# kakaoenterprise/JORLDY

Measured on NVIDIA H100. Metric: env_steps_per_sec, higher is better.
Workload: dtype f32

## Files before the change

include/jorldy_b200.h:

```cpp
#ifndef JORLDY_B200_H
#define JORLDY_B200_H

#include <stdint.h>

#ifdef __cplusplus
#define JB_API extern "C"
#else
#define JB_API
#endif

JB_API int jb_env_classic_reset(int kind, double* phys, float* obs, int32_t* elapsed, int64_t* episode,
                                float* score, const uint8_t* mask, uint64_t seed, uint64_t stream_base,
                                int n, void* stream);
JB_API int jb_env_classic_step(int kind, double* phys, float* obs, int32_t* elapsed, int64_t* episode,
                               float* score, const void* action, int action_kind, float* next_obs,
                               float* reward, float* done, float* stats, int auto_reset, int max_steps,
                               uint64_t seed, uint64_t stream_base, int n, void* stream);

JB_API int jb_gae(const float* reward, const float* done, const float* value, const float* next_value,
                  const float* last_value, int N, int T, float gamma, float lambda, int standardize,
                  float* adv, float* ret, void* stream);

JB_API int
jb_env_synth_reset(float* obs, int32_t* elapsed, int64_t* episode, float* score, uint64_t seed,
// ... 60 lines not shown
                           float* db1, int n1, float* dw2, float* db2, int n2, void* stream);

JB_API int jb_ppo_act_discrete(const float* out, int M, int A, int nout, const float* u, uint64_t seed,
                               uint64_t stream_base, uint64_t ctr, long long* row_ctr, int greedy, int64_t* action,
                               void* stream);
JB_API int jb_ppo_act_continuous(const float* out, int M, int A, int nout, const float* normal, uint64_t seed,
                                 uint64_t stream_base, uint64_t ctr, long long* row_ctr, int greedy, float* action,
                                 void* stream);
JB_API int jb_ppo_prepass_discrete(const float* out, const int32_t* action, int M, int A, int nout, float* value,
                                   float* logp_old, void* stream);
JB_API int jb_ppo_prepass_continuous(const float* out, const float* action, int M, int A, int nout, float* value,
                                     float* logp_old, void* stream);
JB_API int jb_take_minibatch(const int32_t* perm, long long* cursor, int B, int32_t* cur_idx, void* stream);
JB_API int jb_ppo_loss(int continuous, const float* out, const int32_t* idx, const void* action, const float* adv,
                       const float* ret, const float* value_old, const float* logp_old, int B, int A, int nout,
                       float eps_clip, float vf_coef, float ent_coef, float* dout, float* stats, float* acc,
                       void* stream);

JB_API int jb_env_frames_reset(uint8_t* obs, int64_t* fcount, float* score, uint64_t seed, uint64_t stream_base, int n,
                               void* stream);
JB_API int jb_env_frames_step(uint8_t* obs, int64_t* fcount, float* score, uint8_t* next_obs, float* reward, float* done,
                              float* stats, int auto_reset, uint64_t seed, uint64_t stream_base, int n, void* stream);

JB_API int jb_im2col_u8(const uint8_t* x, int B, int C, int H, int W, int KH, int KW, int S, float* col, void* stream);
JB_API int jb_im2col_nhwc(const float* x, int B, int C, int H, int W, int KH, int KW, int S, float* col, void* stream);
JB_API int jb_col2im_nhwc(const float* dcol, int B, int C, int H, int W, int KH, int KW, int S, const float* relu_act,
                          float* dx, void* stream);
JB_API int jb_nhwc_to_nchw(const float* x, int B, int P, int C, float* y, void* stream);
JB_API int jb_nchw_to_nhwc(const float* x, int B, int P, int C, const float* relu_act, float* y, void* stream);

JB_API int jb_ppo_fused_args_size(void);
JB_API int jb_ppo_fused_max_ctas(void);
JB_API int jb_ppo_fused_run(const void* host_args, void* stream);
JB_API int jb_ppo_fused_trace(long long* host_out);

JB_API int jb_q_act(const float* q, int M, int A, float eps, const float* eps_rows, const float* u, uint64_t seed,
                    uint64_t stream_base, long long* row_ctr, int64_t* action, float* q_sel, void* stream);
JB_API int jb_dueling_fwd(const float* adv, const float* val, int B, int A, int K, float* out, void* stream);
JB_API int jb_dueling_bwd(const float* dout, int B, int A, int K, float* dadv, float* dval, void* stream);
JB_API int jb_td_loss(const float* q, const float* q_next, const float* qt_next, const void* action, int action_kind,
                      const float* reward, const float* done, const double* weights, int B, int A, float gamma,
                      float alpha, int n_step, int double_q, int loss_kind, int order, float* dq, double* prio,
                      float* stats, void* stream);

JB_API int jb_c51_loss(const float* logits, const float* next_online, const float* next_target, const void* action,
                       int action_kind, const float* reward, const float* done, const double* weights, const float* z,
                       int B, int A, int K, float gamma, float v_min, float v_max, float alpha, int n_step, int variant,
                       float* dlogits, float* kl, double* prio, float* stats, float* scratch, void* stream);
JB_API int jb_c51_q(const float* logits, const float* z, int M, int A, int K, float* q, void* stream);

JB_API int jb_noisy_make(const float* mu_w, const float* sig_w, const float* mu_b, const float* sig_b, int in_f,
                         int out_f, const float* eps_i, const float* eps_j, uint64_t seed, uint64_t stream_id,
                         long long* draw_ctr, int is_train, float* f_i, float* f_j, float* w_eff, float* b_eff,
                         void* stream);
JB_API int jb_noisy_grad(const float* dw_eff, const float* db_eff, const float* f_i, const float* f_j, int in_f,
                         int out_f, float* dmu_w, float* dsig_w, float* dmu_b, float* dsig_b, void* stream);

JB_API int jb_grad_partials_count(long long P);
JB_API int jb_grad_sumsq(const float* g, long long P, float* partials, long long* step, void* stream);
JB_API int jb_adam_step(float* p, const float* g, float* m, float* v, long long P, const float* lr, double beta1,
                        double beta2, float eps, const long long* step, const float* partials, int n_partials,
                        float max_norm, float* norm_out, void* stream);
JB_API int jb_rmsprop_centered_step(float* p, const float* g, float* square_avg, float* grad_avg, long long P,
                                    const float* lr, double alpha, float eps, const float* partials, int n_partials,
                                    float max_norm, float* norm_out, void* stream);
JB_API int jb_copy_f32(float* dst, const float* src, long long P, void* stream);
// ... 67 lines not shown
```

jorldy_b200/csrc/ppo_fused.cu:

```cuda
#include <cstdlib>
#include "common.cuh"
#include "ppo_rowmath.cuh"
#include "wgmma.cuh"
#include "../../include/jorldy_b200_fused.h"

namespace {

constexpr int NT = 256;
constexpr int PK = 512;
constexpr int MAXD = 16;
constexpr int MAXO = 8;
constexpr int KG = 16;
constexpr int SMALL_FLOATS = 2048;
constexpr int RED_FLOATS = KG * (32 * 36 + 16);
constexpr int JA_ROWS = 256;
constexpr int R2_FLOATS = JA_ROWS * 32;
constexpr int MAX_B = 512;
constexpr int ADAM_IT = 4;
constexpr int PS_FLOATS = (MAXO + 2) * PK;
constexpr int CTR_ROW = 1;
constexpr int CTR_JB = 32;

typedef jb_ppo_fused_args Args;

__device__ __forceinline__ float ldcg(const float* p) { return __ldcg(p); }
__device__ __forceinline__ float4 ldcg4(const float* p) { return __ldcg(reinterpret_cast<const float4*>(p)); }

__device__ __forceinline__ unsigned smem_u32(const void* p) { return (unsigned)__cvta_generic_to_shared(p); }
__device__ __forceinline__ void cp_async4(float* dst, const void* src) {
  asm volatile("cp.async.ca.shared.global [%0], [%1], 4;\n" ::"r"(smem_u32(dst)), "l"(src) : "memory");
}
struct Stager {
  unsigned mbar;
  unsigned bytes;
  unsigned parity;
  __device__ __forceinline__ void init(void* bar) {
    mbar = smem_u32(bar); bytes = 0; parity = 0;
    if (threadIdx.x == 0) {
      asm volatile("mbarrier.init.shared::cta.b64 [%0], 1;\n" ::"r"(mbar) : "memory");
      asm volatile("fence.mbarrier_init.release.cluster;\n" ::: "memory");
    }
  }
  __device__ __forceinline__ void copy(void* dst, const void* src, unsigned nbytes) const {
    asm volatile("cp.async.bulk.shared::cluster.global.mbarrier::complete_tx::bytes [%0], [%1], %2, [%3];\n"
                 ::"r"(smem_u32(dst)), "l"(src), "r"(nbytes), "r"(mbar) : "memory");
  }
  __device__ __forceinline__ void commit() {
    if (bytes && threadIdx.x == 0)
      asm volatile("mbarrier.arrive.expect_tx.shared::cta.b64 _, [%0], %1;\n" ::"r"(mbar), "r"(bytes) : "memory");
    bytes = 0;
  }
  __device__ __forceinline__ void wait() {
    asm volatile(
        "{\n\t"
// ... 217 lines not shown
        "mbarrier.try_wait.parity.shared::cta.b64 p, [%1], %2;\n\t"
        "selp.u32 %0, 1, 0, p;\n\t"
        "}\n" : "=r"(done) : "r"(mbar), "r"(parity) : "memory");
    if (done) return;
    if (clock64() - t0 > (1ll << 32)) asm volatile("trap;\n");
  }
}
__device__ __forceinline__ void mbar_expect_tx(unsigned mbar, unsigned bytes) {
  asm volatile("mbarrier.arrive.expect_tx.shared::cta.b64 _, [%0], %1;\n" ::"r"(mbar), "r"(bytes) : "memory");
}
__device__ __forceinline__ void bulk_g2s(unsigned dst, const void* src, unsigned bytes, unsigned mbar) {
  asm volatile("cp.async.bulk.shared::cluster.global.mbarrier::complete_tx::bytes [%0], [%1], %2, [%3];\n"
               ::"r"(dst), "l"(src), "r"(bytes), "r"(mbar) : "memory");
}
__device__ __forceinline__ float tf32_lo(float x) {
  const float r = x - __uint_as_float(__float_as_uint(x) & 0xFFFFE000u);
  unsigned o;
  asm("cvt.rna.tf32.f32 %0, %1;\n" : "=r"(o) : "f"(r));
  return __uint_as_float(o);
}
constexpr int TC_A_BYTES = 2 * 128 * 128;
constexpr int TC_B_BYTES = 2 * 32 * 128;
constexpr int TC_NA = 3, TC_NB = 5;
constexpr int TC_BAR_WORD = 1664;
constexpr int TC_BAR_JB = TC_NB;
constexpr int TC_NBAR = TC_NB + TC_NA;
constexpr int TC_LD = 36;

__device__ long long g_trace[256 * 48];
#define TR(i) do { if (trace && tid == 0) g_trace[cta * 48 + (i)] = clock64(); } while (0)

struct HeadTab { const float* w[MAXO]; const float* b[MAXO]; float* gw[MAXO]; float* gb[MAXO]; };

template <bool TC, int NA, int ND>
__global__ void __launch_bounds__(NT, 1) ppo_epoch_kernel(Args a, int dsm_floats, int flags ) {
  extern __shared__ __align__(16) float smem[];
  float* s_small = smem;
  float* dsm = smem + SMALL_FLOATS;
  float* R0 = dsm + dsm_floats;
  float* R1 = R0 + RED_FLOATS;
  float* R2 = R1 + RED_FLOATS;
  float* PS = R2 + R2_FLOATS;
  float* xs = s_small;
  float* scr = s_small + 768;
  int* sidx = reinterpret_cast<int*>(s_small + 1024);
  Stager st;
  st.init(s_small + 1056);
  Stager stp;
  stp.init(s_small + 1058);
  float* dvs = s_small + 1088;
  float* hb = s_small + 1600;
  unsigned tc_base = 0;
  unsigned long long tc_g = 0;
  unsigned long long jb_g = 0;
  unsigned long long ja_g = 0;
  const unsigned tc_bar = smem_u32(s_small + TC_BAR_WORD);
  float* tcp = nullptr;
  float* tcs = nullptr;

  const int tid = threadIdx.x, lane = tid & 31, warp = tid >> 5, wg = tid >> 7;
  const unsigned int nctas = gridDim.x;
  const int cta = blockIdx.x;
  const int B = a.B, D = a.D, H = a.H, A = a.A, nout = a.nout;
  const int npol = a.continuous ? 2 * A : A;
  constexpr int NO = 2 * NA + 1 < MAXO ? 2 * NA + 1 : MAXO;
  const int nq = (nout + 3) >> 2;
  const float invB = 1.0f / (float)B;
  const jbppo::HP hp{a.eps_clip, a.vf_coef, a.ent_coef};
  unsigned int epoch = 0;
  const long long step0 = *a.step, cursor0 = *a.cursor;
  const float lr = *a.lr;

  if (TC) {
    tc_base = (smem_u32(R0) + 1023u) & ~1023u;
    tcp = R0 + ((tc_base - smem_u32(R0)) >> 2);
    tcs = tcp + TC_A_BYTES / 4;
    if (tid == 0) {
      for (int i = 0; i < TC_NBAR; ++i) mbar_init(tc_bar + 8u * i, 1);
      asm volatile("fence.mbarrier_init.release.cluster;\n" ::: "memory");
    }
    __syncthreads();
  }
  HeadTab& ht = *reinterpret_cast<HeadTab*>(s_small + 896);
  if (tid == 0) {
    int o = 0;
    for (int g = 0; g < 3; ++g)
      for (int q = 0; q < a.nh[g]; ++q, ++o) {
        ht.w[o] = a.Wh[g] + (size_t)q * H; ht.b[o] = a.bh[g] + q; ht.gw[o] = a.gWh[g] + (size_t)q * H; ht.gb[o] = a.gbh[g] + q;
      }
    for (; o < MAXO; ++o) { ht.w[o] = a.Wh[0]; ht.b[o] = a.bh[0]; ht.gw[o] = a.gWh[0]; ht.gb[o] = a.gbh[0]; }
  }
  __syncthreads();

  const int MT = B / 32, NTL = H / 32, NP = (NTL + 1) >> 1;
  const int nJ1 = TC ? (B >> 7) * NTL : MT * NTL;
  const int nJB = TC ? (H >> 7) * MT : MT * NTL;
  const int nJA = TC ? (H >> 7) * NTL : NTL * NP;
  const int nJC = NTL;
  const int nJD = NTL;
  const int nJ3 = nJB + nJA + nJC + nJD;
  const bool single = B <= JA_ROWS;

  const long long per = (a.P4 + nctas - 1) / nctas;
  const long long lo = (long long)cta * per, hi = min(a.P4, lo + per);
  float4* p4 = reinterpret_cast<float4*>(a.flat);
  const float4* g4 = reinterpret_cast<const float4*>(a.grad);
  float4* m4 = reinterpret_cast<float4*>(a.am);
  float4* v4 = reinterpret_cast<float4*>(a.av);
  double pw1 = pow((double)a.beta1, (double)(step0 + 1)), pw2 = pow((double)a.beta2, (double)(step0 + 1));
  const long long w2_lo = (long long)(a.W2 - a.flat) >> 2, w2_hi = w2_lo + (long long)H * H / 4;
  auto shadow = [&](long long i, float4 v) {
    if (i >= w2_lo && i < w2_hi) {
      const int e = (int)(i - w2_lo) * 4, n = e / H, k = e - n * H;
      *reinterpret_cast<float4*>(&a.W2t[((size_t)(k >> 5) * H + n) * 32 + (k & 31)]) = v;
      if (TC) {
        float* img = a.W2img + ((size_t)(n >> 5) * (H >> 5) + (k >> 5)) * 1024 + (tile_off(n & 31, (k & 31) >> 2) >> 2);
        *reinterpret_cast<float4*>(img) = v;
        *reinterpret_cast<float4*>(img + (size_t)H * H) = make_float4(tf32_lo(v.x), tf32_lo(v.y), tf32_lo(v.z), tf32_lo(v.w));
        const float vv4[4] = {v.x, v.y, v.z, v.w};
#pragma unroll
        for (int q = 0; q < 4; ++q) {
          const int kk = k + q;
          float* t = a.W2Timg + ((size_t)(kk >> 7) * (H >> 5) + (n >> 5)) * 4096 + (tile_off(kk & 127, (n & 31) >> 2) >> 2) + (n & 3);
          t[0] = vv4[q];
          t[(size_t)H * H] = tf32_lo(vv4[q]);
        }
      }
    }
  };
  for (long long i = lo + tid; i < hi; i += NT) shadow(i, p4[i]);
  const float one_m_b1 = 1.f - a.beta1, one_m_b2 = 1.f - a.beta2;

  auto issue_stage = [&](int job, bool b_in_flight) {
    if (job < nJB) {
// ... 329 lines not shown
      tile_reduce<true, true>(acc, R0, outv);
      TR(4);
      {
        float v[4];
#pragma unroll
        for (int r = 0; r < 4; ++r) {
          v[r] = fmaxf(outv[r] + b2v, 0.f);
          a.h2[(size_t)(m0 + warp + 8 * r) * H + n0 + lane] = v[r];
          a.h2t[((size_t)nt * B + m0 + warp + 8 * r) * 32 + lane] = v[r];
        }
        float hv_[16];
        const bool up16 = (lane & 16) != 0;
#pragma unroll
        for (int q = 0; q < 16; ++q) hv_[q] = butterfly_pair(v[q / MAXO] * whr[q % MAXO], v[q / MAXO + 2] * whr[q % MAXO], up16, 16);
        butterfly_level<8>(hv_, lane);
        butterfly_level<4>(hv_, lane);
        butterfly_level<2>(hv_, lane);
        butterfly_level<1>(hv_, lane);
        TR(35);
        const int r = lane >> 3, o = lane & 7;
        if (o < 4 * nq) a.headp[(((size_t)nt * 2 + (o >> 2)) * B + m0 + warp + 8 * r) * 4 + (o & 3)] = o < nout ? hv_[0] : 0.f;
      }
      row_ticket(mt, tid < 32, m0 + tid, tid);
    }
    xs_ready = false;
    TR(5);
    grid_bar(a.barrier, epoch, nctas);
    TR(6);

    stp.bytes = (unsigned)B * (MAXO + 1) * 4u;
    stp.commit();
    if (tid == 0) { stp.copy(dsm, a.dout, (unsigned)B * MAXO * 4u); stp.copy(dvs, a.dv2, (unsigned)B * 4u); }
    int pre_job = -1;
    if (cta < nJ3 && (cta < nJB || prefetchable(cta))) { issue_stage(cta, w2t_pre); pre_job = cta; }
    auto jb_issue_a = [&](int kt4, int nc, unsigned long long g) {
      const unsigned slot = (unsigned)(g % TC_NA);
      const unsigned bar = tc_bar + 8u * (TC_BAR_JB + slot), dst = tc_base + slot * TC_A_BYTES;
      mbar_expect_tx(bar, TC_A_BYTES);
      const float* src = a.W2Timg + ((size_t)kt4 * (H >> 5) + nc) * 4096;
      bulk_g2s(dst, src, 16384u, bar);
      bulk_g2s(dst + 16384u, src + (size_t)H * H, 16384u, bar);
    };
    if (TC && cta >= nJB && cta < nJB + nJA) {
      for (int e = tid; e < B * D; e += NT) { const int m = e / D, i = e - m * D; R2[i * B + m] = ldcg(a.xg + e); }
    }
    if (TC && cta < nJB && tid == 0) {
      jb_issue_a(cta / MT, 0, jb_g);
      if ((H >> 5) > 1) jb_issue_a(cta / MT, 1, jb_g + 1);
    }
    const bool has_next = (s + 1 < a.n_steps) && cta < nJ1;
    int next_r = 0;
    if (TC) { if (has_next) next_r = a.perm[(cursor0 + s + 1) * (long long)B + (cta / NTL) * 128 + (tid & 127)]; }
    else if (has_next && tid < 32) next_r = a.perm[(cursor0 + s + 1) * (long long)B + (cta / NTL) * 32 + tid];

    float c1, c2;
    {
      float p1 = 0.f, p2 = 0.f, ssum = 0.f, esum = 0.f, mr = -INFINITY, mp = INFINITY;
#pragma unroll 1
      for (int b = tid; b < B; b += NT) {
        const float d1 = ldcg(a.rowst + b), d2 = ldcg(a.rowst + B + b);
        p1 = fmaf(d1, d1, p1); p2 = fmaf(d2, d2, p2);
        ssum += ldcg(a.rowst + 2 * B + b); esum += ldcg(a.rowst + 3 * B + b);
        mr = fmaxf(mr, ldcg(a.rowst + 4 * B + b)); mp = fminf(mp, ldcg(a.rowst + 5 * B + b));
      }
      p1 = jb_warp_sum(p1); p2 = jb_warp_sum(p2); ssum = jb_warp_sum(ssum); esum = jb_warp_sum(esum);
      mr = jb_warp_max(mr); mp = jb_warp_min(mp);
      if (lane == 0) { float* q = scr + warp * 8; q[0] = p1; q[1] = p2; q[2] = ssum; q[3] = esum; q[4] = mr; q[5] = mp; }
// ... 36 lines not shown
          scr[96 + 2 * tid + 1] = __uint_as_float((unsigned int)m2);
        }
        __syncthreads();
        TR(40);
        float g1 = 0.f, g2 = 0.f;
        for (int r = 0; r < a.world; ++r) {
          g1 += r == a.rank ? t1 : scr[96 + 2 * r];
          g2 += r == a.rank ? t2 : scr[96 + 2 * r + 1];
        }
        t1 = g1; t2 = g2;
        invBW = invB / (float)a.world;
      }
      c1 = t1 * invBW; c2 = t2 * invBW;
      float w1, w2;
      jbppo::critic_weights(c1, c2, w1, w2);
      stp.wait();
      TR(38);
      for (int b = tid; b < B; b += NT) dsm[b * MAXO + npol] = w1 * dsm[b * MAXO + npol] + w2 * dvs[b];
      if (cta == (int)nctas - 1 && tid == 0) {
        float s3 = 0.f, s4 = 0.f, xr = -INFINITY, xp = INFINITY;
        for (int w = 0; w < NT / 32; ++w) { s3 += scr[w * 8 + 2]; s4 += scr[w * 8 + 3]; xr = fmaxf(xr, scr[w * 8 + 4]); xp = fminf(xp, scr[w * 8 + 5]); }
        a.acc[0] += -s3 * invB;
        a.acc[1] += fmaxf(c1, c2);
        a.acc[2] += -s4 * invB / (a.continuous ? (float)A : 1.f);
        a.acc[3] = fmaxf(a.acc[3], xr);
        a.acc[4] = fminf(a.acc[4], xp);
        a.acc[5] += 1.f;
      }
      __syncthreads();
    }
    TR(7);

    float sq = 0.f;
    for (int job = cta; job < nJ3; job += (int)nctas) {
      __syncthreads();
      TR(8 + min(3, (job - cta) / (int)nctas));
      const int next = job + (int)nctas;
      if (TC && job < nJB) {
        const int kt4 = job / MT, mt = job - kt4 * MT, m0 = mt * 32, kin0 = kt4 * 128, NKC = H >> 5;
        if (job != cta && tid == 0) {
          jb_issue_a(kt4, 0, jb_g);
          if (NKC > 1) jb_issue_a(kt4, 1, jb_g + 1);
        }
        for (int e = tid; e < 32 * MAXD; e += NT) { const int r = e >> 4, i = e & 15; xs[i * 32 + r] = i < D ? ldcg(a.xg + (size_t)(m0 + r) * D + i) : 0.f; }
        const int ml = tid >> 3, c8 = tid & 7;
        const float* drow = &dsm[(m0 + ml) * MAXO];
        float4 hq = ldcg4(a.h2 + (size_t)(m0 + ml) * H + 4 * c8);
        float acc[16];
        for (int nc = 0; nc < NKC; ++nc) {
          const unsigned long long g = jb_g + nc;
          const unsigned slot = (unsigned)(g % TC_NA);
          float4 wr[MAXO];
#pragma unroll
          for (int o = 0; o < MAXO; ++o) wr[o] = o < nout ? *reinterpret_cast<const float4*>(&PS[o * PK + nc * 32 + 4 * c8]) : make_float4(0.f, 0.f, 0.f, 0.f);
          const float4 hcur = hq;
          if (nc + 1 < NKC) hq = ldcg4(a.h2 + (size_t)(m0 + ml) * H + (nc + 1) * 32 + 4 * c8);
          const float4 dv = dh2_quad<NO>(drow, wr, hcur);
          const float4 lo = make_float4(tf32_lo(dv.x), tf32_lo(dv.y), tf32_lo(dv.z), tf32_lo(dv.w));
          const unsigned bbuf = tc_base + TC_NA * TC_A_BYTES + slot * TC_B_BYTES, off = tile_off(ml, c8);
          asm volatile("st.shared.v4.f32 [%0], {%1, %2, %3, %4};\n" ::"r"(bbuf + off), "f"(dv.x), "f"(dv.y), "f"(dv.z), "f"(dv.w) : "memory");
          asm volatile("st.shared.v4.f32 [%0], {%1, %2, %3, %4};\n" ::"r"(bbuf + 4096u + off), "f"(lo.x), "f"(lo.y), "f"(lo.z), "f"(lo.w) : "memory");
          jbwg::wait<0>();
          jbwg::fence_acc(acc);
          asm volatile("fence.proxy.async.shared::cta;\n" ::: "memory");
          __syncthreads();
          if (tid == 0 && nc + 2 < NKC) jb_issue_a(kt4, nc + 2, g + 2);
          mbar_wait(tc_bar + 8u * (TC_BAR_JB + slot), (unsigned)((g / TC_NA) & 1));
          const unsigned aw = tc_base + slot * TC_A_BYTES + (unsigned)wg * 8192u;
          jbwg::fence();
          jbwg::mma3_n32(acc, aw, aw + 16384u, bbuf, bbuf + 4096u, nc == 0);
          jbwg::commit();
        }
        jbwg::wait<0>();
        jbwg::fence_acc(acc);
        __syncthreads();
        jbwg::store_acc_n32(acc, tcs, TC_LD);
        __syncthreads();
        if (prefetchable(next)) { issue_stage(next, false); pre_job = next; }
        {
          const int q = warp & 3, cb = (warp >> 2) * 16, kin = kin0 + q * 32 + lane;
          float rr[16];
#pragma unroll
          for (int c = 0; c < 4; ++c) {
            const float4 t = *reinterpret_cast<const float4*>(&tcs[(q * 32 + lane) * TC_LD + cb + 4 * c]);
            rr[4 * c] = t.x; rr[4 * c + 1] = t.y; rr[4 * c + 2] = t.z; rr[4 * c + 3] = t.w;
          }
          float w1r[ND];
#pragma unroll
          for (int i = 0; i < ND; ++i) w1r[i] = i < D ? ldcg(a.W1 + (size_t)kin * D + i) : 0.f;
          const float b1v = PS[(MAXO + 1) * PK + kin];
          float wacc[ND + 1];
#pragma unroll
          for (int i = 0; i <= ND; ++i) wacc[i] = 0.f;
#pragma unroll
          for (int j = 0; j < 16; ++j) {
            const int ml2 = cb + j;
            float h = 0.f;
#pragma unroll
            for (int i = 0; i < ND; ++i) if (i < D) h = fmaf(xs[i * 32 + ml2], w1r[i], h);
            const float dvv = (h + b1v > 0.f) ? rr[j] : 0.f;
#pragma unroll
            for (int i = 0; i < ND; ++i) if (i < D) wacc[i] = fmaf(dvv, xs[i * 32 + ml2], wacc[i]);
            wacc[ND] += dvv;
          }
          float* sc = tcp + (size_t)(q * 32 + lane) * (MAXD + 1);
          if (warp >= 4) {
#pragma unroll
            for (int i = 0; i <= ND; ++i) if (i < D || i == ND) sc[i < D ? i : MAXD] = wacc[i];
          }
          __syncthreads();
          if (warp < 4) {
// ... 9 lines not shown
        jb_g += (unsigned long long)NKC;
        TR(16);
      } else if (!TC && job < nJB) {
        const int mt = job / NTL, kt = job - mt * NTL;
        const int m0 = mt * 32, k0 = kt * 32;
        if (pre_job != job) issue_stage(job, false);
        const int c4 = (tid & 127) * 4, rh = tid >> 7;
        float4 wr[MAXO];
#pragma unroll
        for (int o = 0; o < MAXO; ++o)
          wr[o] = (o < nout && c4 < H) ? *reinterpret_cast<const float4*>(&PS[o * PK + c4]) : make_float4(0.f, 0.f, 0.f, 0.f);
        if (TC || !(job == cta && nJ1 <= (int)nctas))
          for (int e = tid; e < 32 * MAXD; e += NT) { const int r = e >> 4, i = e & 15; xs[i * 32 + r] = i < D ? ldcg(a.xg + (size_t)(m0 + r) * D + i) : 0.f; }
        float h1m[4];
#pragma unroll
        for (int r = 0; r < 4; ++r)
          asm volatile("ld.global.cg.f32 %0, [%1];\n" : "=f"(h1m[r]) : "l"(a.h1 + ((size_t)kt * B + m0 + warp + 8 * r) * 32 + lane));
        st.wait();
        TR(12);
        if (c4 < H) {
#pragma unroll 4
          for (int r = 0; r < 16; ++r) {
            const int row = rh * 16 + r;
            float4* pa = reinterpret_cast<float4*>(&R0[row * (H + 4) + c4]);
            *pa = dh2_quad<NO>(&dsm[(m0 + row) * MAXO], wr, *pa);
          }
        }
        __syncthreads();
        TR(13);
        float acc[8][8] = {};
        tile_mma<true, false>(R0, R1, H, acc, nullptr);
        __syncthreads();
        TR(14);
        if (prefetchable(next)) { issue_stage(next, false); pre_job = next; }
        float outv[4];
        tile_reduce<true, false>(acc, R0, outv);
        TR(15);
        float wacc[MAXD + 1];
#pragma unroll
        for (int i = 0; i <= MAXD; ++i) wacc[i] = 0.f;
#pragma unroll
        for (int r = 0; r < 4; ++r) {
          const float dv = h1m[r] > 0.f ? outv[r] : 0.f;
          const float* xrow = &xs[warp + 8 * r];
#pragma unroll
          for (int i = 0; i < MAXD; ++i) if (i < D) wacc[i] = fmaf(dv, xrow[i * 32], wacc[i]);
          wacc[MAXD] += dv;
        }
        __syncthreads();
#pragma unroll
        for (int i = 0; i <= MAXD; ++i) if (i < D || i == MAXD) R0[(warp * (MAXD + 1) + i) * 32 + lane] = wacc[i];
        __syncthreads();
        TR(33);
        for (int e = tid; e < 32 * (D + 1); e += NT) {
          const int n = e / (D + 1), i = e - n * (D + 1);
          const int slot = i < D ? i : MAXD;
          float t = R0[(0 * (MAXD + 1) + slot) * 32 + n];
#pragma unroll
          for (int w = 1; w < NT / 32; ++w) t += R0[(w * (MAXD + 1) + slot) * 32 + n];
          a.w1p[((size_t)mt * H + k0) * (D + 1) + e] = t;
        }
        __syncthreads();
        TR(34);
        if (tid == 0) asm volatile("red.release.gpu.global.add.u32 [%0], 1;\n" ::"l"(a.barrier + CTR_JB + kt) : "memory");
        TR(16);
      } else if (TC && job < nJB + nJA) {
        const int j = job - nJB, kt4 = j / NTL, nt = j - kt4 * NTL, k0 = kt4 * 128, n0 = nt * 32, NMC = B >> 5;
// ... 113 lines not shown
        float4 wr[MAXO];
#pragma unroll
        for (int o = 0; o < MAXO; ++o) wr[o] = o < nout ? *reinterpret_cast<const float4*>(&PS[o * PK + n0 + 4 * cg]) : make_float4(0.f, 0.f, 0.f, 0.f);
        const int nhalf = (kt0 + 1 < NTL) ? 2 : 1;
        for (int half = 0; half < nhalf; ++half) {
          const int kt = kt0 + half, k0 = kt * 32;
          const float* Bp = R1 + ((single && half == 1) ? R2_FLOATS : 0);
          float acc[8][8] = {};
          float rs[8] = {0.f, 0.f, 0.f, 0.f, 0.f, 0.f, 0.f, 0.f};
          for (int mp = 0; mp < B; mp += JA_ROWS) {
            const int kp = min(JA_ROWS, B - mp);
            if (!single || half == 0) {
              if (single) {
                if (pre_job != job) issue_stage(job, false);
              } else {
                __syncthreads();
                stage_block(st, R2, a.h2t + ((size_t)nt * B + mp) * 32, kp);
                stage_block(st, R1, a.h1 + ((size_t)kt * B + mp) * 32, kp);
                st.commit();
              }
              st.wait();
              TR(17);
              for (int m = rl; m < kp; m += 32) {
                float4* pa = reinterpret_cast<float4*>(&R2[m * 32 + 4 * cg]);
                *pa = dh2_quad<NO>(&dsm[(mp + m) * MAXO], wr, *pa);
              }
              __syncthreads();
              TR(18);
            }
            tile_mma<false, false>(R2, Bp, kp, acc, kt == 0 ? rs : nullptr);
          }
          __syncthreads();
          TR(19);
          if (half == nhalf - 1 && prefetchable(next)) { issue_stage(next, false); pre_job = next; }
          float outv[4];
          tile_reduce<false, false>(acc, R0, outv);
          TR(20);
#pragma unroll
          for (int r = 0; r < 4; ++r) {
            a.gW2[(size_t)(n0 + warp + 8 * r) * H + k0 + lane] = outv[r];
            sq = fmaf(outv[r], outv[r], sq);
          }
          if (kt == 0) {
            const int grp = tid >> 4, t = tid & 15, tx = t & 3, ty = t >> 2;
            __syncthreads();
            if (tx == 0) {
#pragma unroll
              for (int i = 0; i < 8; ++i) R0[grp * 32 + ty * 8 + i] = rs[i];
            }
            __syncthreads();
            if (tid < 32) {
              float v = 0.f;
#pragma unroll
              for (int g = 0; g < KG; ++g) v += R0[g * 32 + tid];
              a.gb2[n0 + tid] = v;
              sq = fmaf(v, v, sq);
            }
            __syncthreads();
          }
        }
        TR(21);
      } else if (job < nJB + nJA + nJC) {
        const int jt = job - nJB - nJA;
        const int j0 = jt * 32;
        float hacc[MAXO];
#pragma unroll
        for (int o = 0; o < MAXO; ++o) hacc[o] = 0.f;
        for (int mp = 0; mp < B; mp += JA_ROWS) {
          const int kp = min(JA_ROWS, B - mp);
          if (!(mp == 0 && pre_job == job)) { __syncthreads(); stage_block(st, R2, a.h2t + ((size_t)jt * B + mp) * 32, kp); st.commit(); }
          st.wait();
          if (!TC) TR(39);
#pragma unroll 4
          for (int m = warp; m < kp; m += NT / 32) {
            const float hvv = R2[m * 32 + lane];
            const float4 d0 = *reinterpret_cast<const float4*>(&dsm[(mp + m) * MAXO]);
            const float4 d1 = *reinterpret_cast<const float4*>(&dsm[(mp + m) * MAXO + 4]);
            hacc[0] = fmaf(d0.x, hvv, hacc[0]); hacc[1] = fmaf(d0.y, hvv, hacc[1]); hacc[2] = fmaf(d0.z, hvv, hacc[2]);
            hacc[3] = fmaf(d0.w, hvv, hacc[3]); hacc[4] = fmaf(d1.x, hvv, hacc[4]); hacc[5] = fmaf(d1.y, hvv, hacc[5]);
            hacc[6] = fmaf(d1.z, hvv, hacc[6]); hacc[7] = fmaf(d1.w, hvv, hacc[7]);
          }
        }
        __syncthreads();
        if (prefetchable(next)) { issue_stage(next, false); pre_job = next; }
        float* red = R0;
#pragma unroll
        for (int o = 0; o < MAXO; ++o) red[(warp * MAXO + o) * 32 + lane] = hacc[o];
        __syncthreads();
        if (warp == 0) {
#pragma unroll
          for (int o = 0; o < MAXO; ++o) {
            if (o < nout) {
              float t = red[(0 * MAXO + o) * 32 + lane];
              for (int r = 1; r < NT / 32; ++r) t += red[(r * MAXO + o) * 32 + lane];
              ht.gw[o][j0 + lane] = t;
              sq = fmaf(t, t, sq);
            }
          }
        }
        if (jt == 0) {
          __syncthreads();
          const int o = tid & 7, part = tid >> 3;
          float t = 0.f;
          for (int m = part; m < B; m += NT / 8) t += dsm[m * MAXO + o];
          red[part * MAXO + o] = t;
          __syncthreads();
          if (tid < MAXO) {
            float tt = 0.f;
            for (int q = 0; q < NT / 8; ++q) tt += red[q * MAXO + tid];
            if (tid < nout) { *ht.gb[tid] = tt; sq = fmaf(tt, tt, sq); }
          }
        }
        if (!TC) TR(30);
      } else {
        const int kt = job - nJB - nJA - nJC, k0 = kt * 32;
        if (tid == 0) {
          const unsigned int target = (unsigned int)MT * (unsigned int)(s + 1);
          unsigned int v;
          do {
            asm volatile("ld.relaxed.gpu.global.u32 %0, [%1];\n" : "=r"(v) : "l"(a.barrier + CTR_JB + kt) : "memory");
          } while (v < target);
          asm volatile("fence.acq_rel.gpu;\n" ::: "memory");
        }
        __syncthreads();
        if (!TC) TR(31);
        for (int e = tid; e < 32 * (D + 1); e += NT) {
          const int n = e / (D + 1), i = e - n * (D + 1);
          float t = ldcg(a.w1p + (size_t)k0 * (D + 1) + e);
          for (int mt = 1; mt < MT; ++mt) t += ldcg(a.w1p + ((size_t)mt * H + k0) * (D + 1) + e);
          if (i < D) a.gW1[(size_t)(k0 + n) * D + i] = t; else a.gb1[k0 + n] = t;
          sq = fmaf(t, t, sq);
        }
        if (!TC) TR(32);
      }
    }
    TR(22);
    if (a.world == 1) {
      const float tot = block_sum(sq, scr + 64);
      if (tid == 0) a.partials[cta] = tot;
    }
    if (!TC && has_next && tid < 32) sidx[tid] = next_r;
    float4 pp[ADAM_IT], mm[ADAM_IT], vv[ADAM_IT];
#pragma unroll
    for (int it = 0; it < ADAM_IT; ++it) {
      const long long i = lo + tid + it * NT;
      if (i < hi) { pp[it] = __ldcg(p4 + i); mm[it] = __ldcg(m4 + i); vv[it] = __ldcg(v4 + i); }
    }
    TR(23);
    grid_bar(a.barrier, epoch, nctas);
    TR(24);

    {
      float4 gg[ADAM_IT];
      if (a.world == 1) {
#pragma unroll
        for (int it = 0; it < ADAM_IT; ++it) {
          const long long i = lo + tid + it * NT;
          if (i < hi) gg[it] = __ldcg(g4 + i);
        }
      } else {
        const unsigned int target = a.xbase + (unsigned int)s + 1u;
        unsigned int* abortf = a.barrier + CTR_ABORT;
        const long long q4 = (a.P4 + a.world - 1) / a.world, c4 = (q4 + nctas - 1) / nctas;
        bool ok = true;
        for (int q = 0; q < a.world; ++q) {
          if (q == a.rank) continue;
          const long long sl_lo = (long long)q * q4, sl_hi = min(a.P4, sl_lo + q4);
          const long long ch_lo = sl_lo + (long long)cta * c4, ch_hi = min(sl_hi, ch_lo + c4);
          unsigned long long* inbox = reinterpret_cast<unsigned long long*>(a.peer[q] + a.xllin_off) + ((size_t)a.rank * q4) * 4;
          for (long long i = ch_lo + tid; i < ch_hi; i += NT) ll_store4(inbox + (i - sl_lo) * 4, __ldcg(g4 + i), target);
// ... 91 lines not shown
        const long long i = lo + tid + it * NT;
        if (i < hi) {
          upd(pp[it].x, gg[it].x, mm[it].x, vv[it].x); upd(pp[it].y, gg[it].y, mm[it].y, vv[it].y);
          upd(pp[it].z, gg[it].z, mm[it].z, vv[it].z); upd(pp[it].w, gg[it].w, mm[it].w, vv[it].w);
          p4[i] = pp[it]; m4[i] = mm[it]; v4[i] = vv[it];
          shadow(i, pp[it]);
        }
      }
      for (long long i = lo + tid + (long long)ADAM_IT * NT; i < hi; i += NT) {
        float4 p_ = __ldcg(p4 + i), m_ = __ldcg(m4 + i), v_ = __ldcg(v4 + i);
        float4 g_;
        if (a.world > 1) {
          if (!ll_load4(reinterpret_cast<const unsigned long long*>(a.peer[a.rank] + a.xgred_off) + (size_t)i * 4, a.xbase + (unsigned int)s + 1u, g_, a.barrier + CTR_ABORT)) a.acc[7] = 1.f;
        } else g_ = __ldcg(g4 + i);
        upd(p_.x, g_.x, m_.x, v_.x); upd(p_.y, g_.y, m_.y, v_.y); upd(p_.z, g_.z, m_.z, v_.z); upd(p_.w, g_.w, m_.w, v_.w);
        p4[i] = p_; m4[i] = m_; v4[i] = v_;
        shadow(i, p_);
      }
      if (has_next) {
        if (!TC) {
#pragma unroll
          for (int q = 0; q < 2; ++q) { const int e = tid + q * NT; xs[(e & 15) * 32 + (e >> 4)] = xv[q]; }
        }
        xs_ready = true;
      }
    }
    TR(26);
    grid_bar(a.barrier, epoch, nctas);
    TR(27);
  }
  if (cta == 0 && tid == 0) { *a.step = step0 + a.n_steps; *a.cursor = cursor0 + a.n_steps; }
}

static int dsm_floats_for(int B) { return B * MAXO; }
static size_t fused_smem(int B) { return sizeof(float) * (size_t)(SMALL_FLOATS + dsm_floats_for(B) + 2 * RED_FLOATS + R2_FLOATS + PS_FLOATS); }

static const void* fused_fn(bool tc, int A, int D) {
  const int na = A <= 2 ? 0 : (A <= 4 ? 1 : 2), nd = D <= 4 ? 0 : 1;
  static const void* const tab[4][3] = {
      {(const void*)ppo_epoch_kernel<false, 2, 4>, (const void*)ppo_epoch_kernel<false, 4, 4>, (const void*)ppo_epoch_kernel<false, 8, 4>},
      {(const void*)ppo_epoch_kernel<false, 2, 16>, (const void*)ppo_epoch_kernel<false, 4, 16>, (const void*)ppo_epoch_kernel<false, 8, 16>},
      {(const void*)ppo_epoch_kernel<true, 2, 4>, (const void*)ppo_epoch_kernel<true, 4, 4>, (const void*)ppo_epoch_kernel<true, 8, 4>},
      {(const void*)ppo_epoch_kernel<true, 2, 16>, (const void*)ppo_epoch_kernel<true, 4, 16>, (const void*)ppo_epoch_kernel<true, 8, 16>}};
  return tab[(tc ? 2 : 0) + nd][na];
}

static int fused_max_ctas(int B, bool tc = false, int A = 8, int D = 16) {
  int dev = 0, sms = 0, per_sm = 0;
  cudaGetDevice(&dev);
  cudaDeviceGetAttribute(&sms, cudaDevAttrMultiProcessorCount, dev);
  const size_t smem = fused_smem(B);
  if (smem > 227 * 1024) return 0;
  const void* fn = fused_fn(tc, A, D);
  cudaFuncSetAttribute(fn, cudaFuncAttributeMaxDynamicSharedMemorySize, (int)smem);
  cudaOccupancyMaxActiveBlocksPerMultiprocessor(&per_sm, fn, NT, smem);
  return sms * (per_sm > 0 ? 1 : 0);
}

}

JB_API int jb_ppo_fused_args_size(void) { return (int)sizeof(jb_ppo_fused_args); }

JB_API int jb_ppo_fused_max_ctas(void) { return fused_max_ctas(256); }

JB_API int jb_ppo_fused_trace(long long* host_out) {
  return cudaMemcpyFromSymbol(host_out, g_trace, sizeof(long long) * 256 * 48) == cudaSuccess ? JB_OK : JB_ERR_CUDA;
}

JB_API int jb_ppo_fused_run(const void* host_args, void* stream) {
  if (!host_args) return JB_ERR_INVALID;
  Args a = *reinterpret_cast<const Args*>(host_args);
  if (a.B <= 0 || a.B % 32 || a.B > MAX_B || a.H <= 0 || a.H % 32 || a.H > PK || a.D <= 0 || a.D > MAXD || a.nout <= 0 ||
      a.nout > MAXO || a.A <= 0 || a.A > jbppo::MAX_A || a.n_steps <= 0 || a.P4 <= 0)
    return JB_ERR_INVALID;
  bool tc = false;
  if (const char* e = getenv("JB_FUSED_TC")) tc = atoi(e) != 0;
  tc = tc && a.B % 128 == 0 && a.H % 128 == 0 && a.W2img != nullptr && a.W2Timg != nullptr;
  int ctas = fused_max_ctas(a.B, tc, a.A, a.D);
  if (ctas <= 0) return JB_ERR_INVALID;
  if (ctas > NT) ctas = NT;
  if (a.world < 1 || a.world > 8 || a.rank < 0 || a.rank >= a.world) return JB_ERR_INVALID;
  if (a.world > 1) {
    const long long q4 = (a.P4 + a.world - 1) / a.world;
    if (a.peer[a.rank] != a.grad || a.xllin_off < a.P4 * 4 || a.xgred_off < a.xllin_off + 8 * a.world * q4 ||
        a.xflag_off < a.xgred_off + 8 * a.P4 || (a.xllin_off & 7) || (a.xgred_off & 7) || (a.xflag_off & 3) || ctas > JB_X_MAX_CTAS)
      return JB_ERR_INVALID;
    for (int r = 0; r < a.world; ++r) if (!a.peer[r]) return JB_ERR_INVALID;
  }
  cudaStream_t s = (cudaStream_t)stream;
  if (cudaMemsetAsync(a.barrier, 0, 64 * sizeof(unsigned int), s) != cudaSuccess) return JB_ERR_CUDA;
  const size_t smem = fused_smem(a.B);
  int dsm_floats = dsm_floats_for(a.B);
  int flags = 0;
  if (const char* e = getenv("JB_FUSED_SKIP")) flags = atoi(e);
  void* kargs[] = {&a, &dsm_floats, &flags};
  cudaError_t e = cudaLaunchCooperativeKernel(const_cast<void*>(fused_fn(tc, a.A, a.D)), dim3(ctas), dim3(NT), kargs, smem, s);
  if (e != cudaSuccess) { cudaGetLastError(); return JB_ERR_CUDA; }
  return JB_OK;
}
```

Baseline: 2.037 million.

## Balance phase-3 small jobs across CTAs with a host-built weighted job map

Replaces the round-robin job assignment in the fused PPO backward phase with a host-computed per-CTA job list. Head-gradient jobs stay round-robin, while the small bias/W1-reduction jobs go greedily to the least-loaded CTA using estimated cost weights. The list is passed as a grid-constant parameter and linked in shared memory. Gradient-norm accumulation moves out of the job loop into a separate pass gated by a global completion counter, which adds a spin-wait and extra reads in exchange for evening out per-CTA work.

After: 2.003 million, median of 6. 1.6% lower.

```diff
diff --git a/include/jorldy_b200.h b/include/jorldy_b200.h
--- a/include/jorldy_b200.h
+++ b/include/jorldy_b200.h
@@ -116,6 +116,7 @@
 JB_API int jb_ppo_fused_args_size(void);
 JB_API int jb_ppo_fused_max_ctas(void);
 JB_API int jb_ppo_fused_run(const void* host_args, void* stream);
+JB_API int jb_ppo_fused_job_map(int B, int H, int tc, int nctas, int16_t* off, int16_t* job);
 JB_API int jb_ppo_fused_trace(long long* host_out);
 
 JB_API int jb_q_act(const float* q, int M, int A, float eps, const float* eps_rows, const float* u, uint64_t seed,
diff --git a/jorldy_b200/csrc/ppo_fused.cu b/jorldy_b200/csrc/ppo_fused.cu
--- a/jorldy_b200/csrc/ppo_fused.cu
+++ b/jorldy_b200/csrc/ppo_fused.cu
@@ -20,6 +20,7 @@
 constexpr int PS_FLOATS = (MAXO + 2) * PK;
 constexpr int CTR_ROW = 1;
 constexpr int CTR_JB = 32;
+constexpr int CTR_SMALL = 48;
 
 typedef jb_ppo_fused_args Args;
 
@@ -303,8 +304,14 @@
 
 struct HeadTab { const float* w[MAXO]; const float* b[MAXO]; float* gw[MAXO]; float* gb[MAXO]; };
 
+constexpr int MAX_CTAS = NT;
+constexpr int MAX_J3 = (MAX_B / 32) * (PK / 32) + (PK / 32) * (PK / 64) + 2 * (PK / 32);
+struct JobMap { int16_t off[MAX_CTAS + 1]; int16_t job[MAX_J3]; };
+static_assert(4 * (TC_BAR_WORD + 2 * TC_NBAR) + 3 * (MAX_J3 + 1) <= 4 * SMALL_FLOATS, "a CTA's job list fits behind the mbarriers");
+
 template <bool TC, int NA, int ND>
-__global__ void __launch_bounds__(NT, 1) ppo_epoch_kernel(Args a, int dsm_floats, int flags ) {
+__global__ void __launch_bounds__(NT, 1) ppo_epoch_kernel(Args a, const __grid_constant__ JobMap jm, int dsm_floats,
+                                                          int flags ) {
   extern __shared__ __align__(16) float smem[];
   float* s_small = smem;
   float* dsm = smem + SMALL_FLOATS;
@@ -371,6 +378,16 @@
   const int nJD = NTL;
   const int nJ3 = nJB + nJA + nJC + nJD;
   const bool single = B <= JA_ROWS;
+  int16_t* jnext = reinterpret_cast<int16_t*>(s_small + TC_BAR_WORD + 2 * TC_NBAR);
+  int8_t* jslot = reinterpret_cast<int8_t*>(jnext + MAX_J3 + 1);
+  if (tid == 0) {
+    int prev = MAX_J3;
+    for (int k = jm.off[cta]; k < jm.off[cta + 1]; ++k) {
+      jnext[prev] = jm.job[k]; prev = jm.job[k];
+      jslot[prev] = (int8_t)(8 + min(3, k - jm.off[cta]));
+    }
+    jnext[prev] = (int16_t)nJ3;
+  }
 
   const long long per = (a.P4 + nctas - 1) / nctas;
   const long long lo = (long long)cta * per, hi = min(a.P4, lo + per);
@@ -766,7 +783,7 @@
     stp.commit();
     if (tid == 0) { stp.copy(dsm, a.dout, (unsigned)B * MAXO * 4u); stp.copy(dvs, a.dv2, (unsigned)B * 4u); }
     int pre_job = -1;
-    if (cta < nJ3 && (cta < nJB || prefetchable(cta))) { issue_stage(cta, w2t_pre); pre_job = cta; }
+    if (const int j0 = jnext[MAX_J3]; j0 < nJB || prefetchable(j0)) { issue_stage(j0, w2t_pre); pre_job = j0; }
     auto jb_issue_a = [&](int kt4, int nc, unsigned long long g) {
       const unsigned slot = (unsigned)(g % TC_NA);
       const unsigned bar = tc_bar + 8u * (TC_BAR_JB + slot), dst = tc_base + slot * TC_A_BYTES;
@@ -869,10 +886,13 @@
     TR(7);
 
     float sq = 0.f;
-    for (int job = cta; job < nJ3; job += (int)nctas) {
+    for (int job = jnext[MAX_J3]; job < nJ3; job = jnext[job]) {
       __syncthreads();
-      TR(8 + min(3, (job - cta) / (int)nctas));
-      const int next = job + (int)nctas;
+      TR(jslot[job]);
+      auto prefetch_next = [&]() {
+        const int next = jnext[job];
+        if (prefetchable(next)) { issue_stage(next, false); pre_job = next; }
+      };
       if (TC && job < nJB) {
         const int kt4 = job / MT, mt = job - kt4 * MT, m0 = mt * 32, kin0 = kt4 * 128, NKC = H >> 5;
         if (job != cta && tid == 0) {
@@ -913,7 +933,7 @@
         __syncthreads();
         jbwg::store_acc_n32(acc, tcs, TC_LD);
         __syncthreads();
-        if (prefetchable(next)) { issue_stage(next, false); pre_job = next; }
+        prefetch_next();
         {
           const int q = warp & 3, cb = (warp >> 2) * 16, kin = kin0 + q * 32 + lane;
           float rr[16];
@@ -989,7 +1009,7 @@
         tile_mma<true, false>(R0, R1, H, acc, nullptr);
         __syncthreads();
         TR(14);
-        if (prefetchable(next)) { issue_stage(next, false); pre_job = next; }
+        prefetch_next();
         float outv[4];
         tile_reduce<true, false>(acc, R0, outv);
         TR(15);
@@ -1169,7 +1189,7 @@
           }
           __syncthreads();
           TR(19);
-          if (half == nhalf - 1 && prefetchable(next)) { issue_stage(next, false); pre_job = next; }
+          if (half == nhalf - 1) prefetch_next();
           float outv[4];
           tile_reduce<false, false>(acc, R0, outv);
           TR(20);
@@ -1219,7 +1239,7 @@
           }
         }
         __syncthreads();
-        if (prefetchable(next)) { issue_stage(next, false); pre_job = next; }
+        prefetch_next();
         float* red = R0;
 #pragma unroll
         for (int o = 0; o < MAXO; ++o) red[(warp * MAXO + o) * 32 + lane] = hacc[o];
@@ -1231,7 +1251,6 @@
               float t = red[(0 * MAXO + o) * 32 + lane];
               for (int r = 1; r < NT / 32; ++r) t += red[(r * MAXO + o) * 32 + lane];
               ht.gw[o][j0 + lane] = t;
-              sq = fmaf(t, t, sq);
             }
           }
         }
@@ -1245,7 +1264,7 @@
           if (tid < MAXO) {
             float tt = 0.f;
             for (int q = 0; q < NT / 8; ++q) tt += red[q * MAXO + tid];
-            if (tid < nout) { *ht.gb[tid] = tt; sq = fmaf(tt, tt, sq); }
+            if (tid < nout) *ht.gb[tid] = tt;
           }
         }
         if (!TC) TR(30);
@@ -1266,13 +1285,44 @@
           float t = ldcg(a.w1p + (size_t)k0 * (D + 1) + e);
           for (int mt = 1; mt < MT; ++mt) t += ldcg(a.w1p + ((size_t)mt * H + k0) * (D + 1) + e);
           if (i < D) a.gW1[(size_t)(k0 + n) * D + i] = t; else a.gb1[k0 + n] = t;
-          sq = fmaf(t, t, sq);
         }
         if (!TC) TR(32);
       }
+    }
+    __syncthreads();
+    if (tid == 0) {
+      unsigned int n = 0;
+      for (int j = jnext[MAX_J3]; j < nJ3; j = jnext[j]) n += j >= nJB + nJA;
+      if (n) asm volatile("red.release.gpu.global.add.u32 [%0], %1;\n" ::"l"(a.barrier + CTR_SMALL), "r"(n) : "memory");
     }
     TR(22);
     if (a.world == 1) {
+      for (int j = cta; j < nJ3; j += (int)nctas) {
+        if (j < nJB + nJA) continue;
+        if (tid == 0) {
+          const unsigned int target = (unsigned int)(nJC + nJD) * (unsigned int)(s + 1);
+          unsigned int v;
+          do {
+            asm volatile("ld.relaxed.gpu.global.u32 %0, [%1];\n" : "=r"(v) : "l"(a.barrier + CTR_SMALL) : "memory");
+          } while (v < target);
+          asm volatile("fence.acq_rel.gpu;\n" ::: "memory");
+        }
+        __syncthreads();
+        if (j < nJB + nJA + nJC) {
+          const int j0 = (j - nJB - nJA) * 32;
+          if (warp == 0) {
+            for (int o = 0; o < nout; ++o) { const float t = ldcg(ht.gw[o] + j0 + lane); sq = fmaf(t, t, sq); }
+          }
+          if (j0 == 0 && tid < nout) { const float t = ldcg(ht.gb[tid]); sq = fmaf(t, t, sq); }
+        } else {
+          const int k0 = (j - nJB - nJA - nJC) * 32;
+          for (int e = tid; e < 32 * (D + 1); e += NT) {
+            const int n = e / (D + 1), i = e - n * (D + 1);
+            const float t = ldcg(i < D ? a.gW1 + (size_t)(k0 + n) * D + i : a.gb1 + k0 + n);
+            sq = fmaf(t, t, sq);
+          }
+        }
+      }
       const float tot = block_sum(sq, scr + 64);
       if (tid == 0) a.partials[cta] = tot;
     }
@@ -1430,6 +1480,35 @@
   if (cta == 0 && tid == 0) { *a.step = step0 + a.n_steps; *a.cursor = cursor0 + a.n_steps; }
 }
 
+static int p3_job_map(int B, int H, bool tc, int nctas, int16_t* off, int16_t* job) {
+  if (B <= 0 || B % 32 || B > MAX_B || H <= 0 || H % 32 || H > PK || nctas < 1 || nctas > MAX_CTAS) return -1;
+  if (tc && (B % 128 || H % 128)) return -1;
+  const int MT = B / 32, NTL = H / 32, NP = (NTL + 1) >> 1;
+  const int nJB = tc ? (H >> 7) * MT : MT * NTL, nJA = tc ? (H >> 7) * NTL : NTL * NP;
+  const int nH = nJB + nJA, nJC = NTL, nJ3 = nH + nJC + NTL;
+  if (!off || !job) return nJ3;
+  const long long wJB = 7600, wJA = 6300LL * B / 256, wJC = 1600LL * B / 256, wJD = 2100LL * B / 256;
+  long long load[MAX_CTAS];
+  int cnt[MAX_CTAS], owner[2 * (PK / 32)];
+  for (int c = 0; c < nctas; ++c) { load[c] = 0; cnt[c] = 0; }
+  for (int j = 0; j < nH; ++j) { load[j % nctas] += j < nJB ? wJB : wJA; ++cnt[j % nctas]; }
+  for (int j = nH; j < nJ3; ++j) {
+    int best = 0;
+    for (int c = 1; c < nctas; ++c) if (load[c] < load[best]) best = c;
+    load[best] += j < nH + nJC ? wJC : wJD;
+    ++cnt[best];
+    owner[j - nH] = best;
+  }
+  off[0] = 0;
+  for (int c = 0; c < nctas; ++c) {
+    int k = off[c];
+    for (int j = c; j < nH; j += nctas) job[k++] = (int16_t)j;
+    for (int j = nH; j < nJ3; ++j) if (owner[j - nH] == c) job[k++] = (int16_t)j;
+    off[c + 1] = (int16_t)k;
+  }
+  return nJ3;
+}
+
 static int dsm_floats_for(int B) { return B * MAXO; }
 static size_t fused_smem(int B) { return sizeof(float) * (size_t)(SMALL_FLOATS + dsm_floats_for(B) + 2 * RED_FLOATS + R2_FLOATS + PS_FLOATS); }
 
@@ -1460,6 +1539,11 @@
 JB_API int jb_ppo_fused_args_size(void) { return (int)sizeof(jb_ppo_fused_args); }
 
 JB_API int jb_ppo_fused_max_ctas(void) { return fused_max_ctas(256); }
+
+JB_API int jb_ppo_fused_job_map(int B, int H, int tc, int nctas, int16_t* off, int16_t* job) {
+  const int n = p3_job_map(B, H, tc != 0, nctas, off, job);
+  return n < 0 ? JB_ERR_INVALID : n;
+}
 
 JB_API int jb_ppo_fused_trace(long long* host_out) {
   return cudaMemcpyFromSymbol(host_out, g_trace, sizeof(long long) * 256 * 48) == cudaSuccess ? JB_OK : JB_ERR_CUDA;
@@ -1488,10 +1572,12 @@
   cudaStream_t s = (cudaStream_t)stream;
   if (cudaMemsetAsync(a.barrier, 0, 64 * sizeof(unsigned int), s) != cudaSuccess) return JB_ERR_CUDA;
   const size_t smem = fused_smem(a.B);
+  JobMap jm;
+  if (p3_job_map(a.B, a.H, tc, ctas, jm.off, jm.job) < 0) return JB_ERR_INVALID;
   int dsm_floats = dsm_floats_for(a.B);
   int flags = 0;
   if (const char* e = getenv("JB_FUSED_SKIP")) flags = atoi(e);
-  void* kargs[] = {&a, &dsm_floats, &flags};
+  void* kargs[] = {&a, &jm, &dsm_floats, &flags};
   cudaError_t e = cudaLaunchCooperativeKernel(const_cast<void*>(fused_fn(tc, a.A, a.D)), dim3(ctas), dim3(NT), kargs, smem, s);
   if (e != cudaSuccess) { cudaGetLastError(); return JB_ERR_CUDA; }
   return JB_OK;
```
